# blackjax-devs/blackjax

Measured on AMD Instinct MI355X. Metric: chain-leapfrog-steps/sec (whole node), 65 536 chains x 1 024-dim diag-mass HMC, higher is better.
Workload: dtype f32

## Files before the change

blackjax_amd/_lib.py:

```python
from __future__ import annotations

import ctypes
import os
from ctypes import POINTER, c_char_p, c_float, c_int, c_int64, c_uint32, c_void_p

_HERE = os.path.dirname(os.path.abspath(__file__))
LIB_PATH = os.path.join(_HERE, "libbjxhip.so")

_f32p = c_void_p
_u8p = c_void_p

SIGNATURES = {
    "bjx_abi_version": [],
    "bjx_keys_split": [c_uint32, c_uint32, c_int64, c_int64, POINTER(c_uint32)],
    "bjx_rng_normal": [c_void_p, c_uint32, c_uint32, c_int64, c_int64, c_int64, _f32p],
    "bjx_rng_uniform": [c_void_p, c_uint32, c_uint32, c_int64, c_int64, _f32p],
    "bjx_rng_key_probe": [c_void_p, c_uint32, c_uint32, c_int64, _f32p, _f32p, c_int64, c_void_p],
    "bjx_log1p_device_check": [c_void_p, c_uint32, c_void_p],
    "bjx_hmc_momentum_diag": [c_void_p, c_uint32, c_uint32, c_int64, c_int64, c_int64, c_int64, _f32p,
                              c_int64, _f32p, _f32p],
    "bjx_hmc_momentum_kick_diag": [c_void_p, c_uint32, c_uint32, c_int64, c_int64, c_int64, c_int64, _f32p,
                                   c_int64, c_float, _f32p, _f32p, _f32p, _f32p, _f32p, _f32p, _f32p],
    "bjx_leapfrog_diag": [c_void_p, c_int64, c_int64, c_int, c_float, _f32p, _f32p, c_int64,
                          _f32p, _f32p, _f32p, _f32p, _f32p],
# ... 62 lines not shown
                                 _f32p, _f32p, _f32p, _f32p, _f32p, _u8p, _u8p, _f32p, _f32p, _f32p, _f32p,
                                 _f32p, c_void_p],
    "bjx_pc_matvec_t": [c_void_p, c_int64, c_int64, _f32p, c_int64, _f32p, _f32p],
    "bjx_hmc_momentum_dense_pc": [c_void_p, c_uint32, c_uint32, c_int64, c_int64, c_int64, c_int64,
                                  _f32p, _f32p, c_int64, _f32p, _f32p, _f32p, _f32p],
    "bjx_leapfrog_dense_pc": [c_void_p, c_int64, c_int64, c_int, c_float, _f32p, _f32p, c_int64, _f32p,
                              _f32p, _f32p, _f32p, _f32p],
    "bjx_hmc_finish_dense_pc": [c_void_p, c_uint32, c_uint32, c_int64, c_int64, c_int64, c_int64,
                                c_float, _f32p, _f32p, c_int64, c_float,
                                _f32p, _f32p, _f32p, _f32p, _f32p, _f32p, _f32p, _f32p,
                                _f32p, _f32p, _f32p, _f32p, _f32p, _f32p, _f32p, _u8p, _u8p, _f32p],
    "bjx_welford_update_dense": [c_void_p, c_int64, c_int64, c_int64, _f32p, _f32p, _f32p, _f32p,
                                 _f32p],
    "bjx_welford_final_dense": [c_void_p, c_int64, c_int64, c_int64, c_float, _f32p, _f32p, c_int,
                                _f32p],
    "bjx_da_init": [c_void_p, c_int64, c_int, _f32p, _f32p, _f32p, _f32p, _f32p, _f32p],
    "bjx_da_update": [c_void_p, c_int64, c_int64, c_float, c_float, c_float, c_float, _f32p, _f32p,
                      _f32p, _f32p, _f32p, _f32p, _f32p, _f32p, _f32p],
    "bjx_exp": [c_void_p, c_int64, _f32p, _f32p],
    "bjx_welford_update_diag": [c_void_p, c_int64, c_int64, c_int64, _f32p, _f32p, _f32p, _f32p, _f32p],
    "bjx_welford_final_diag": [c_void_p, c_int64, c_int64, c_int64, c_float, _f32p, _f32p, c_int64,
                               _f32p],
    "bjx_target_diag_gaussian": [c_void_p, c_int64, c_int64, _f32p, _f32p, _f32p, _f32p],
    "bjx_target_neal_funnel": [c_void_p, c_int64, c_int64, _f32p, _f32p, _f32p],
    "bjx_target_ar1_gaussian": [c_void_p, c_int64, c_int64, c_float, c_float, c_float, _f32p,
                                _f32p, _f32p],
}



class NutsDesc(ctypes.Structure):

    _fields_ = [
        ("N", c_int64), ("D", c_int64), ("max_depth", ctypes.c_int32), ("reserved", ctypes.c_int32),
        ("imm", c_void_p), ("imm_stride", c_int64), ("eps_per_chain", c_void_p),
        ("eps", c_float), ("divergence_threshold", c_float),
        ("key0", c_uint32), ("key1", c_uint32), ("chain_offset", c_int64), ("step_fold", c_int64),
        ("q0", c_void_p), ("g0", c_void_p), ("p0", c_void_p),
        ("Lq", c_void_p), ("Lp", c_void_p), ("Lg", c_void_p),
        ("Rq", c_void_p), ("Rp", c_void_p), ("Rg", c_void_p),
        ("msum", c_void_p), ("Smsum", c_void_p),
        ("Pq", c_void_p), ("Pg", c_void_p), ("Sq", c_void_p), ("Sg", c_void_p),
        ("ckpt_r", c_void_p), ("ckpt_rs", c_void_p),
        ("fs", c_void_p), ("is_", c_void_p),
        ("Mdense", c_void_p), ("Mdense_stride", c_int64), ("v0", c_void_p),
        ("Lv", c_void_p), ("Rv", c_void_p), ("ckpt_v", c_void_p),
# ... 235 lines not shown
```

blackjax_amd/_util.py:

```python
from __future__ import annotations

import threading
import weakref
from typing import Callable

import torch

_VG_CACHE: "weakref.WeakKeyDictionary" = weakref.WeakKeyDictionary()
_CAPTURE_LOCK = threading.RLock()
_CAPTURE_TLS = threading.local()
_GRAVEYARD: list = []


class LockedGraph(torch.cuda.CUDAGraph):

    def __del__(self):
        try:
            if getattr(_CAPTURE_TLS, "depth", 0) > 0:
                _GRAVEYARD.append(self)
                return
            with _CAPTURE_LOCK:
                self.reset()
        except Exception:
            pass
# ... 94 lines not shown
                    return lp_a, g_a
            return tgt(q)
        lp, g = first if first is not None else _autograd(q)
        ew[key] = _try_elementwise(logdensity_fn, q, lp, g)
        return lp, g

    def vg(q):
        if mode["kind"] == "autograd":
            return _autograd_or_elementwise(q)
        if mode["kind"] == "pair":
            return logdensity_fn(q)
        qg = q.detach().requires_grad_(True)
        with torch.enable_grad():
            out = logdensity_fn(qg)
            if isinstance(out, (tuple, list)) and len(out) == 2:
                mode["kind"] = "pair"
                lp, g = out[0].detach(), out[1].detach()
                del out
                return lp, g
            mode["kind"] = "autograd"
            g = _grad(out, qg)
        return _autograd_or_elementwise(q, first=(out.detach(), g))

    vg._bjx_elementwise = ew
    vg._bjx_value_and_grad = True
    try:
        _VG_CACHE[logdensity_fn] = vg
    except TypeError:
        pass
    return vg


_WARNED_AUTOGRAD: set = set()
_RECHECK_AT = (16, 256)
_RECHECK_EVERY = 4096


def _close(a, b) -> bool:
    a, b = a.float(), b.float()
    fin = torch.isfinite(b)
    scale = float(b[fin].abs().max()) if bool(fin.any()) else 1.0
    same_nonfinite = bool(((a == b) | (torch.isnan(a) & torch.isnan(b)))[~fin].all())
    return same_nonfinite and bool(((a - b)[fin].abs() <= 1e-4 * max(scale, 1e-30)).all())


def no_trace(logdensity_fn: Callable) -> Callable:
# ... 114 lines not shown
        raise RuntimeError(
            f"{name} lives on {x.device}: blackjax_amd runs on ROCm device tensors only "
            "(there is no CPU fallback)"
        )
    if x.dtype != torch.float32:
        raise TypeError(f"{name} must be float32, got {x.dtype}")
    return x.contiguous()


def eval_logdensity(vg: Callable, q: torch.Tensor):
    logp, g = vg(q)
    if logp.dtype != torch.float32:
        logp = logp.float()
    if g.dtype != torch.float32:
        g = g.float()
    if g.shape != q.shape or logp.shape != q.shape[:1]:
        raise ValueError(
            f"logdensity_fn must return logp of shape {tuple(q.shape[:1])} and grad of shape "
            f"{tuple(q.shape)}; got {tuple(logp.shape)} and {tuple(g.shape)}"
        )
    return logp.contiguous(), g.contiguous()


def step_size_args(step_size, n_chains: int, device):
    if isinstance(step_size, torch.Tensor):
        if step_size.ndim == 0 and not step_size.is_cuda:
            return float(step_size), None
        t = step_size.to(device=device, dtype=torch.float32)
        if t.ndim == 0:
            t = t.expand(n_chains)
        if t.shape != (n_chains,):
            raise ValueError(f"per-chain step_size must have shape ({n_chains},), got {tuple(t.shape)}")
        return 0.0, t.contiguous()
    return float(step_size), None
```

blackjax_amd/csrc/bjx_targets.hip:

```cpp
#include "../../include/bjx_hip.h"
#include "bjx_device.h"
#include "bjx_host.h"
#include "bjx_targets_dev.h"

using namespace bjx;

namespace {

constexpr int kBlock = 256;
constexpr int kWavesPerBlock = kBlock / BJX_WAVE;

__device__ __forceinline__ int64_t wave_row0() {
  return (int64_t)blockIdx.x * kWavesPerBlock + (threadIdx.x >> 6);
}
__device__ __forceinline__ int64_t wave_row_stride() { return (int64_t)gridDim.x * kWavesPerBlock; }

template <int VEC, bool NT = false>
__global__ void __launch_bounds__(kBlock)
k_diag_gaussian(int64_t N, int64_t D, const float* __restrict__ iv, const float* __restrict__ q,
                float* __restrict__ logp, float* __restrict__ g) {
  const int lane = threadIdx.x & 63;
  for (int64_t r = wave_row0(); r < N; r += wave_row_stride()) {
    const int64_t base = r * D;
    double acc = 0.0;
// ... 15 lines not shown
          if (j < D) {
            F4 gg{-(qq[u].x * vv[u].x), -(qq[u].y * vv[u].y), -(qq[u].z * vv[u].z), -(qq[u].w * vv[u].w)};
            acc += (double)qq[u].x * (double)gg.x;
            acc += (double)qq[u].y * (double)gg.y;
            acc += (double)qq[u].z * (double)gg.z;
            acc += (double)qq[u].w * (double)gg.w;
            st4_t<NT>(g + base + j, gg);
          }
        }
      }
    } else {
      for (int64_t j = lane; j < D; j += 64) {
        const float qq = q[base + j];
        const float gg = -(qq * iv[j]);
        acc += (double)qq * (double)gg;
        g[base + j] = gg;
      }
    }
    acc = wave_sum(acc);
    if (lane == 0) logp[r] = (float)(0.5 * acc);
  }
}

template <int G>
__global__ void __launch_bounds__(kBlock)
k_diag_gaussian_short(int64_t N, int64_t D, const float* __restrict__ iv, const float* __restrict__ q,
                      float* __restrict__ logp, float* __restrict__ g) {
  constexpr int R = BJX_WAVE / G;
  const int lane = threadIdx.x & 63;
  const int sub = lane / G, gl = lane % G;
  for (int64_t r0 = wave_row0() * R; r0 < N; r0 += wave_row_stride() * R) {
    const int64_t r = r0 + sub;
    const bool valid = r < N;
    double acc = 0.0;
    if (valid) {
      const int64_t base = r * D;
      for (int64_t j = (int64_t)gl * 4; j < D; j += G * 4) {
        const F4 qq = ld4(q + base + j), vv = ld4(iv + j);
        const F4 gg{-(qq.x * vv.x), -(qq.y * vv.y), -(qq.z * vv.z), -(qq.w * vv.w)};
        acc += (double)qq.x * (double)gg.x;
        acc += (double)qq.y * (double)gg.y;
        acc += (double)qq.z * (double)gg.z;
        acc += (double)qq.w * (double)gg.w;
        st4(g + base + j, gg);
      }
    }
// ... 87 lines not shown
    hipLaunchKernelGGL(k_diag_gaussian_short<8>, dim3(bjx_row_grid((N + 7) / 8, kWavesPerBlock)), block, 0,
                       (hipStream_t)stream, N, D, inv_var, q, logp_out, g_out);
  else if (bjx_vec4_ok(D, inv_var, q, g_out) && D <= 64)
    hipLaunchKernelGGL(k_diag_gaussian_short<16>, dim3(bjx_row_grid((N + 3) / 4, kWavesPerBlock)), block, 0,
                       (hipStream_t)stream, N, D, inv_var, q, logp_out, g_out);
  else if (bjx_vec4_ok(D, inv_var, q, g_out) && D <= 128)
    hipLaunchKernelGGL(k_diag_gaussian_short<32>, dim3(bjx_row_grid((N + 1) / 2, kWavesPerBlock)), block, 0,
                       (hipStream_t)stream, N, D, inv_var, q, logp_out, g_out);
  else if (bjx_vec4_ok(D, inv_var, q, g_out)) {
    static const int nt_mode = [] { const char* e = getenv("BJX_LF_NT"); return e ? atoi(e) : -1; }();
    const bool nt = nt_mode < 0 ? N * D * 8 > ((int64_t)256 << 20) : nt_mode != 0;
    if (nt)
      hipLaunchKernelGGL((k_diag_gaussian<4, true>), grid, block, 0, (hipStream_t)stream, N, D, inv_var, q,
                         logp_out, g_out);
    else
      hipLaunchKernelGGL((k_diag_gaussian<4, false>), grid, block, 0, (hipStream_t)stream, N, D, inv_var, q,
                         logp_out, g_out);
  } else
    hipLaunchKernelGGL(k_diag_gaussian<1>, grid, block, 0, (hipStream_t)stream, N, D, inv_var, q,
                       logp_out, g_out);
  return bjx_check_launch("bjx_target_diag_gaussian");
}

int bjx_target_neal_funnel(void* stream, int64_t N, int64_t D, const float* q, float* logp_out,
                           float* g_out) {
  BJX_CHECK_ARG(N >= 0 && D >= 2, "bjx_target_neal_funnel: bad arguments");
  if (N == 0) return 0;
  BJX_CHECK_ARG(q && logp_out && g_out, "bjx_target_neal_funnel: bad arguments");
  const dim3 grid(bjx_row_grid(N, kWavesPerBlock));
  hipStream_t st = (hipStream_t)stream;
  if (bjx_vec4_ok(D, q, g_out) && D <= 1024) {
    const dim3 wgrid((unsigned)(N < ((int64_t)1 << 20) ? N : ((int64_t)1 << 20)));
    if (D <= 256) hipLaunchKernelGGL(k_neal_funnel_v4<1>, wgrid, dim3(64), 0, st, N, D, q, logp_out, g_out);
    else if (D <= 512) hipLaunchKernelGGL(k_neal_funnel_v4<2>, wgrid, dim3(64), 0, st, N, D, q, logp_out, g_out);
    else hipLaunchKernelGGL(k_neal_funnel_v4<4>, wgrid, dim3(64), 0, st, N, D, q, logp_out, g_out);
  } else {
    hipLaunchKernelGGL(k_neal_funnel, grid, dim3(kBlock), 0, st, N, D, q, logp_out, g_out);
  }
  return bjx_check_launch("bjx_target_neal_funnel");
}

int bjx_target_ar1_gaussian(void* stream, int64_t N, int64_t D, float diag_edge, float diag_mid,
                            float off, const float* q, float* logp_out, float* g_out) {
  BJX_CHECK_ARG(N >= 0 && D >= 2, "bjx_target_ar1_gaussian: bad arguments");
  if (N == 0) return 0;
  BJX_CHECK_ARG(q && logp_out && g_out, "bjx_target_ar1_gaussian: bad arguments");
// ... 7 lines not shown
```

blackjax_amd/csrc/bjx_traj_dev.h:

```cpp
#pragma once

#include "bjx_device.h"
#include "bjx_targets_dev.h"

namespace bjx {

struct TrajArgs {
  Key key;
  int64_t off, fold, N, D, L;
  float eps_s;
  const float* eps_pc;
  const float* imm;
  int64_t imm_stride;
  float thr;
  const float* params;
  const float *q0, *logp0, *g0;
  float *p0_out, *q1_out, *p_end_out, *logp1_out, *g1_out;
  float *q_out, *logp_out, *g_out, *acc_rate_out, *energy_out;
  uint8_t *is_acc_out, *is_div_out;
};

static_assert(sizeof(TrajArgs) == 216, "blackjax_amd/rtc.py mirrors this struct field for field (TrajArgs)");

struct FunnelTarget {
// ... 151 lines not shown
  }
}

template <int NI, class Target>
__device__ __forceinline__ void target_rows(int64_t N, int64_t D, const float* params, const float* q,
                                            float* logp, float* grad) {
  const int lane = threadIdx.x & 63;
  const int waves = blockDim.x >> 6;
  for (int64_t r = (int64_t)blockIdx.x * waves + (threadIdx.x >> 6); r < N; r += (int64_t)gridDim.x * waves) {
    typename Target::template Ctx<NI> ctx;
    Target::template init<NI>(ctx, D, params);
    F4 x[NI], g[NI];
    float lp = 0.0f;
#pragma unroll
    for (int k = 0; k < NI; ++k) {
      const int64_t j = ((int64_t)lane + 64 * k) * 4;
      if (j < D) x[k] = ld4(q + r * D + j);
    }
    Target::template eval<NI>(ctx, D, params, x, true, g, lp);
    target_store<NI>(D, g, lp, logp + r, grad + r * D);
  }
}

}
```

blackjax_amd/elementwise.py:

```python
from __future__ import annotations

import math
import operator
from typing import Callable

import torch

__all__ = ["from_elementwise", "ElementwiseSource"]


class _E:

    __slots__ = ("v", "d")

    def __init__(self, v: str, d):
        self.v, self.d = v, d


class _R:

    __slots__ = ("coef", "const")

    def __init__(self, coef: dict, const: float = 0.0):
        self.coef, self.const = coef, float(const)
# ... 358 lines not shown
          const float xs[4] = {{xq[u].x, xq[u].y, xq[u].z, xq[u].w}}; {p_unpack_u}
          float gs[4];
#pragma unroll
          for (int e = 0; e < 4; ++e) {{
            const float x = xs[e]; {p_decl}
            {body}
            gs[e] = {g_expr};
            {acc_add_rows}
          }}
          st4(gr + j, F4{{gs[0], gs[1], gs[2], gs[3]}});
        }});
    }} else {{
      for (int64_t j = lane; j < D; j += 64) {{
        const float x = qr[j]; {p_scalar}
        {body}
        gr[j] = {g_expr};
        {acc_add_rows}
      }}
    }}
    const float lp = (float)({lp_expr});
    if (lane == 0) logp[r] = lp;
  }}
}}
"""
    params = torch.stack(gen.params).contiguous() if gen.params else None
    src = ElementwiseSource(source, params, len(used),
                            f"{len(gen.lines)} fp32 ops per element, {n_p} parameter vector(s), {len(used)} row sum(s)")
    src.rows_source = rows_source
    return src


class _Wrap(torch.nn.Module):

    def __init__(self, fn):
        super().__init__()
        self._fn = fn

    def forward(self, q):
        return self._fn(q)


ROWS_TU = """#include "bjx_traj_dev.h"
using namespace bjx;
%(source)s
"""

# ... 14 lines not shown
```

blackjax_amd/hmc.py:

```python
from __future__ import annotations

from typing import Callable, NamedTuple

import torch

from . import _lib, integrators, metrics
from ._util import (new_graph, record_graph, check_batch, eval_logdensity, is_capturable, step_size_args, value_and_grad,
                    warn_eager_driver)
from .base import SamplingAlgorithm
from .random import key_spec

__all__ = ["HMCState", "HMCInfo", "IntegratorState", "init", "flip_momentum", "build_kernel", "as_top_level_api"]


class HMCState(NamedTuple):

    position: torch.Tensor
    logdensity: torch.Tensor
    logdensity_grad: torch.Tensor


class IntegratorState(NamedTuple):

    position: torch.Tensor
    momentum: torch.Tensor
    logdensity: torch.Tensor
    logdensity_grad: torch.Tensor


class HMCInfo(NamedTuple):

# ... 161 lines not shown
    return int(v)


_IC_WORKING_SET_BYTES = 192 << 20


def auto_chain_block(n_chains: int, dim: int, arrays: int = 3) -> int:
    blk = (_IC_WORKING_SET_BYTES // (4 * int(arrays) * max(int(dim), 1))) // 1024 * 1024
    if blk < 1024 or blk >= n_chains:
        return int(n_chains)
    return int(blk)


class _GraphedTrajectory:

    def __init__(self, n, D, L, vg, imm_per_chain, device, owner=None):
        self.n, self.D, self.L = n, D, L
        self.owner = owner
        self.Wq = torch.empty((n, D), dtype=torch.float32, device=device)
        self.Wp = torch.empty((n, D), dtype=torch.float32, device=device)
        self.eps = torch.ones(n, dtype=torch.float32, device=device)
        self.imm = torch.ones((n, D) if imm_per_chain else (D,), dtype=torch.float32, device=device)
        self.imm_stride = D if imm_per_chain else 0
        self.Wq.zero_()
        self.Wp.zero_()
        self._vg = vg
        side = torch.cuda.Stream(device=device)
        side.wait_stream(torch.cuda.current_stream(device))
        with torch.cuda.stream(side):
            self._body()
        torch.cuda.current_stream(device).wait_stream(side)
        torch.cuda.synchronize(device)
        self.graph = new_graph()
        with record_graph(self.graph):
            self.logp, self.g = self._body()

    def _body(self):
        stream = _lib.current_stream()
        logp, g = eval_logdensity(self._vg, self.Wq)
        for _ in range(self.L - 1):
            _lib.call("bjx_leapfrog_diag", stream, self.n, self.D, 2, 0.0, self.eps.data_ptr(),
                      self.imm.data_ptr(), self.imm_stride, self.Wq.data_ptr(), self.Wp.data_ptr(),
                      g.data_ptr(), self.Wq.data_ptr(), self.Wp.data_ptr())
            del logp, g
            logp, g = eval_logdensity(self._vg, self.Wq)
        return logp, g


_SIDE_STREAMS: dict = {}


def _side_streams(dev, n):
    pool = _SIDE_STREAMS.setdefault(dev.index, [])
    while len(pool) < n:
        pool.append(torch.cuda.Stream(device=dev))
    return pool[:n]


def build_kernel(integrator=integrators.velocity_verlet, divergence_threshold: float = 1000,
                 build_proposal=None, *, chain_block=None, use_graph="auto", streams="auto"):
    if use_graph not in (True, False, "auto"):
        raise ValueError("use_graph must be True, False or 'auto'")
    thr = float(divergence_threshold)
    if build_proposal is multinomial_hmc_proposal:
        integrators.check_supported(integrator, allow_general=True)
        return _build_mhmc_kernel(thr, integrator.coefficients[0::2], integrator.coefficients[1::2])
    if build_proposal not in (None, hmc_proposal):
        raise NotImplementedError(
# ... 50 lines not shown
                cb = N
        blk = N if not cb or cb >= N else int(cb)
        n_blocks = (N + blk - 1) // blk if N else 0
        fn_id = id(logdensity_fn)
        if (use_graph == "auto" and L >= 2 and N > 0 and metric.kind == "diag" and not general
                and blk * D <= (1 << 21) and is_capturable(logdensity_fn)
                and fn_id not in not_capturable):
            gkey = (min(blk, N), D, L, fn_id, metric.imm_stride != 0, dev.index)
            seen[gkey] = seen.get(gkey, 0) + 1
            try:
                if gkey not in graphs and seen[gkey] >= 2 and len(graphs) < 8:
                    graphs[gkey] = _GraphedTrajectory(min(blk, N), D, L, vg, metric.imm_stride != 0, dev,
                                                      owner=logdensity_fn)
                graphed = gkey in graphs
            except RuntimeError:
                not_capturable[fn_id] = logdensity_fn
                torch.cuda.synchronize(dev)
        if (use_graph == "auto" and L >= 2 and N > 0 and metric.kind == "diag" and not general
                and blk * D <= (1 << 21) and not is_capturable(logdensity_fn)):
            warn_eager_driver(logdensity_fn, "hmc")
        single = n_blocks <= 1 and not graphed
        q_end = torch.empty_like(q0) if L > 0 else q0
        p_work = torch.empty_like(q0) if (L > 0 and not graphed) else None
        g_end = torch.empty_like(q0) if (L > 0 and not single) else None
        logp_end = torch.empty_like(logp0) if (L > 0 and not single) else None
        if L == 0:
            g_end, logp_end = g0, logp0

        def block_args(b):
            s, e = b * blk, min(N, (b + 1) * blk)
            sl = slice(s, e)
            if metric.kind == "dense_pc":
                m = metric._replace(imm=metric.imm[sl], mass_sqrt_t=metric.mass_sqrt_t[sl])
            else:
                m = metric if metric.imm_stride == 0 else metric._replace(imm=metric.imm[sl])
            return e - s, sl, m, (None if eps_pc is None else eps_pc[sl]), off + s

        fused_first = (metric.kind == "diag" and L > 0 and not graphed and not general and D > 128 and _FUSE_FIRST)

        def launch_first(b, stream_):
            n, sl, m, eb, boff = block_args(b)
            _lib.call("bjx_hmc_momentum_kick_diag", stream_, k0, k1, boff, fold, n, D, m.imm.data_ptr(),
                      m.imm_stride, eps, _lib.ptr(eb), q0[sl].data_ptr(), g0[sl].data_ptr(),
                      p0[sl].data_ptr(), ke0[sl].data_ptr(), q_end[sl].data_ptr(), p_work[sl].data_ptr())

        def run_block(b):
            nonlocal g_end, logp_end
            stream = _lib.current_stream()
            n, sl, m, eb, boff = block_args(b)
            if fused_first:
                q, p = q_end[sl], p_work[sl]
                launch_first(b, stream)
            elif m.kind == "diag":
                _lib.call("bjx_hmc_momentum_diag", stream, k0, k1, boff, fold, n, D, m.imm.data_ptr(),
                          m.imm_stride, p0[sl].data_ptr(), ke0[sl].data_ptr())
            else:
                from . import dense

                dense.momentum(stream, m, k0, k1, boff, fold, n, D, p0[sl], ke0[sl])

            if L == 0:
                q, p, logp, g = q0[sl], p0[sl], logp0[sl], g0[sl]
                eps_fin, eps_pc_fin = 0.0, None
            elif graphed:
                gkey = (n, D, L, fn_id, m.imm_stride != 0, dev.index)
                ctx = graphs.get(gkey)
                if ctx is None:
                    ctx = graphs[gkey] = _GraphedTrajectory(n, D, L, vg, m.imm_stride != 0, dev,
                                                            owner=logdensity_fn)
                if eb is None:
                    ctx.eps.fill_(eps)
                else:
                    ctx.eps.copy_(eb)
                ctx.imm.copy_(m.imm)
                _launch_leapfrog(stream, m, n, D, 1, eps, eb, q0[sl], p0[sl], g0[sl], ctx.Wq, ctx.Wp)
                ctx.graph.replay()
                q, p, logp, g = ctx.Wq, ctx.Wp, ctx.logp, ctx.g
                eps_fin, eps_pc_fin = eps, eb
            elif general:
                q, p = q_end[sl], p_work[sl]

                def stage(n_k, ka, kb, a_c, q_in, p_in, g_in, p_out):
                    if m.kind == "diag":
                        _lib.call("bjx_leapfrog_diag_coef", stream, n, D, n_k, ka, kb, a_c, eps, _lib.ptr(eb),
                                  m.imm.data_ptr(), m.imm_stride, q_in.data_ptr(), p_in.data_ptr(),
                                  g_in.data_ptr(), q.data_ptr(), p_out.data_ptr(), None, 0)
                        return p_out
                    from . import dense

                    return dense.leapfrog_coef(stream, m, n, D, n_k, ka, kb, a_c, eps, eb, q_in, p_in,
                                               g_in, q, p_out)

                first = True
                for _ in range(L):
                    for si, a_c in enumerate(drift_c):
                        if first:
                            p = stage(1, kick_c[0], 0.0, a_c, q0[sl], p0[sl], g0[sl], p)
                            first = False
                        elif si == 0:
                            p = stage(2, kick_c[-1], kick_c[0], a_c, q, p, g, p)
                        else:
                            p = stage(1, kick_c[si], 0.0, a_c, q, p, g, p)
                        logp, g = eval_logdensity(vg, q)
                        yield
                        stream = _lib.current_stream()
                eps_fin, eps_pc_fin = eps, eb
            else:
                if not fused_first:
                    q, p = q_end[sl], p_work[sl]
                    p = _launch_leapfrog(stream, m, n, D, 1, eps, eb, q0[sl], p0[sl], g0[sl], q, p)
                logp, g = eval_logdensity(vg, q)
                for _ in range(L - 1):
                    yield
                    stream = _lib.current_stream()
                    p = _launch_leapfrog(stream, m, n, D, 2, eps, eb, q, p, g, q, p)
                    logp, g = eval_logdensity(vg, q)
                yield
                stream = _lib.current_stream()
                eps_fin, eps_pc_fin = eps, eb

            if m.kind == "diag" and general:
                _lib.call("bjx_hmc_finish_diag_coef", stream, k0, k1, boff, fold, n, D, kick_c[-1],
                          eps_fin, _lib.ptr(eps_pc_fin), m.imm.data_ptr(), m.imm_stride, thr,
                          q0[sl].data_ptr(), logp0[sl].data_ptr(), g0[sl].data_ptr(),
                          ke0[sl].data_ptr(), q.data_ptr(), logp.data_ptr(), g.data_ptr(),
                          p.data_ptr(), p_end[sl].data_ptr(), q_new[sl].data_ptr(),
                          logp_new[sl].data_ptr(), g_new[sl].data_ptr(), acc_rate[sl].data_ptr(),
                          is_acc[sl].data_ptr(), is_div[sl].data_ptr(), energy[sl].data_ptr())
            elif m.kind == "diag":
                _lib.call("bjx_hmc_finish_diag", stream, k0, k1, boff, fold, n, D, eps_fin,
                          _lib.ptr(eps_pc_fin), m.imm.data_ptr(), m.imm_stride, thr,
                          q0[sl].data_ptr(), logp0[sl].data_ptr(), g0[sl].data_ptr(),
                          ke0[sl].data_ptr(), q.data_ptr(), logp.data_ptr(), g.data_ptr(),
                          p.data_ptr(), p_end[sl].data_ptr(), q_new[sl].data_ptr(),
                          logp_new[sl].data_ptr(), g_new[sl].data_ptr(), acc_rate[sl].data_ptr(),
                          is_acc[sl].data_ptr(), is_div[sl].data_ptr(), energy[sl].data_ptr())
            elif general:
                from . import dense

                dense.finish_coef(stream, m, k0, k1, boff, fold, n, D, kick_c[-1], eps_fin, eps_pc_fin, thr,
                                  q0[sl], logp0[sl], g0[sl], ke0[sl], q, logp, g, p, p_end[sl], q_new[sl],
                                  logp_new[sl], g_new[sl], acc_rate[sl], is_acc[sl], is_div[sl], energy[sl])
            else:
                from . import dense

                dense.finish(stream, m, k0, k1, boff, fold, n, D, eps_fin, eps_pc_fin, thr, q0[sl],
                             logp0[sl], g0[sl], ke0[sl], q, logp, g, p, p_end[sl], q_new[sl],
                             logp_new[sl], g_new[sl], acc_rate[sl], is_acc[sl], is_div[sl],
                             energy[sl])
            if L > 0:
                if single:
                    g_end, logp_end = g, logp
                else:
                    g_end[sl].copy_(g)
                    logp_end[sl].copy_(logp)
                    if graphed:
                        q_end[sl].copy_(q)


        ns = 1 if (graphed or n_blocks <= 1) else min(int(n_streams), n_blocks)
        if ns <= 1:
            for b in range(n_blocks):
                for _ in run_block(b):
                    pass
        else:
            main = torch.cuda.current_stream(dev)
            pool = _side_streams(dev, ns)
            for st_ in pool:
                st_.wait_stream(main)
            for w0 in range(0, n_blocks, ns):
                active = [(run_block(b), pool[b - w0]) for b in range(w0, min(w0 + ns, n_blocks))]
                while active:
                    for item in list(active):
                        with torch.cuda.stream(item[1]):
                            try:
                                next(item[0])
                            except StopIteration:
                                active.remove(item)
            for st_ in pool:
                main.wait_stream(st_)
# ... 87 lines not shown
```

blackjax_amd/rtc.py:

```python
from __future__ import annotations

import ctypes
import os

_HERE = os.path.dirname(os.path.abspath(__file__))
CSRC = os.path.join(_HERE, "csrc")
ARCH = "gfx950"

_rtc = None
_hip = None


def _librtc():
    global _rtc
    if _rtc is None:
        _rtc = ctypes.CDLL("libhiprtc.so")
        _rtc.hiprtcGetErrorString.restype = ctypes.c_char_p
    return _rtc


def _libhip():
    global _hip
    if _hip is None:
        _hip = ctypes.CDLL("libamdhip64.so")
# ... 79 lines not shown
                ("L", ctypes.c_int64), ("eps_s", ctypes.c_float), ("eps_pc", ctypes.c_void_p),
                ("imm", ctypes.c_void_p), ("imm_stride", ctypes.c_int64), ("thr", ctypes.c_float),
                ("params", ctypes.c_void_p), ("q0", ctypes.c_void_p), ("logp0", ctypes.c_void_p),
                ("g0", ctypes.c_void_p), ("p0_out", ctypes.c_void_p), ("q1_out", ctypes.c_void_p),
                ("p_end_out", ctypes.c_void_p), ("logp1_out", ctypes.c_void_p), ("g1_out", ctypes.c_void_p),
                ("q_out", ctypes.c_void_p), ("logp_out", ctypes.c_void_p), ("g_out", ctypes.c_void_p),
                ("acc_rate_out", ctypes.c_void_p), ("energy_out", ctypes.c_void_p),
                ("is_acc_out", ctypes.c_void_p), ("is_div_out", ctypes.c_void_p)]


TARGET_TU = """#include "bjx_traj_dev.h"
using namespace bjx;
// ---- user source
%(source)s
// ---- kernels around it
#define BJX_RTC_KERNELS(NI_)                                                                              \\
  extern "C" __global__ void __launch_bounds__(256) bjx_rtc_traj_##NI_(TrajArgs a) {                      \\
    hmc_trajectory_rows<NI_, %(struct)s>(a);                                                              \\
  }                                                                                                       \\
  extern "C" __global__ void __launch_bounds__(256) bjx_rtc_eval_##NI_(long long N, long long D,          \\
                                                                       const float* params, const float* q, \\
                                                                       float* logp, float* grad) {        \\
    target_rows<NI_, %(struct)s>(N, D, params, q, logp, grad);                                            \\
  }
BJX_RTC_KERNELS(1)
BJX_RTC_KERNELS(2)
BJX_RTC_KERNELS(4)
"""


def ni_for(dim: int) -> int:
    return 1 if dim <= 256 else (2 if dim <= 512 else 4)


NUTS_TU = """#include "bjx_traj_dev.h"
using namespace bjx;
// ---- user source
%(source)s
// ---- the engine's NUTS device code around it
#define BJX_RTC_USER_TARGET %(struct)s
#include "bjx_nuts_tick_dev.h"
#define BJX_RTC_NUTS(NI_, FULL_, NAME_)                                                                      \\
  extern "C" __global__ void __launch_bounds__(64) __attribute__((amdgpu_waves_per_eu(2)))                   \\
  NAME_(bjx_nuts_t nt, bjx_nuts_async_t ax, float* qf, float* logp_f, float* gf) {                           \\
    const int64_t n_rows = async_n_rows(ax);                                                                 \\
    for (int64_t b = blockIdx.x; b < n_rows; b += gridDim.x)                                                 \\
# ... 13 lines not shown
```

blackjax_amd/targets.py:

```python
from __future__ import annotations

import numpy as np
import torch

from . import _lib
from ._util import check_batch


class _Target:
    _bjx_value_and_grad = True
    _bjx_returns_pair = True
    _bjx_capturable = True

    def _alloc(self, q):
        q = check_batch(q, "q")
        return q, torch.empty(q.shape[0], dtype=torch.float32, device=q.device), torch.empty_like(q)


class DiagGaussian(_Target):
    def __init__(self, inv_var: torch.Tensor):
        self.inv_var = check_batch(inv_var, "inv_var")

    def _bjx_fused_target(self, dim: int):
        if dim > 128 and tuple(self.inv_var.shape) == (dim,):
            return 2, self.inv_var
        return None

    def __call__(self, q):
        q, logp, g = self._alloc(q)
        N, D = q.shape
        if self.inv_var.shape != (D,):
            raise ValueError(f"inv_var has shape {tuple(self.inv_var.shape)}, expected ({D},)")
        _lib.call("bjx_target_diag_gaussian", _lib.current_stream(), N, D, self.inv_var.data_ptr(),
                  q.data_ptr(), logp.data_ptr(), g.data_ptr())
        return logp, g


class NealFunnel(_Target):
    def _bjx_fused_target(self, dim: int):
        return 1, None

    def __call__(self, q):
        q, logp, g = self._alloc(q)
        N, D = q.shape
        _lib.call("bjx_target_neal_funnel", _lib.current_stream(), N, D, q.data_ptr(),
                  logp.data_ptr(), g.data_ptr())
        return logp, g


class AR1Gaussian(_Target):
    def __init__(self, rho: float, dim: int):
        self.rho, self.dim = float(rho), int(dim)
        c = np.float32(1.0 / (1.0 - self.rho * self.rho))
        self.d_edge = float(np.float32(1.0) * c)
        self.d_mid = float(np.float32(1.0 + self.rho * self.rho) * c)
        self.off = float(np.float32(-self.rho) * c)

    def covariance(self, device) -> torch.Tensor:
        i = torch.arange(self.dim, device=device)
        return (self.rho ** (i[:, None] - i[None, :]).abs().double()).float()

    def __call__(self, q):
        q, logp, g = self._alloc(q)
        N, D = q.shape
        if D != self.dim:
            raise ValueError(f"expected dim {self.dim}, got {D}")
        _lib.call("bjx_target_ar1_gaussian", _lib.current_stream(), N, D, self.d_edge, self.d_mid,
                  self.off, q.data_ptr(), logp.data_ptr(), g.data_ptr())
        return logp, g


class DeviceTarget(_Target):

    def __init__(self, source: str, params: torch.Tensor | None = None, struct: str = "Target"):
        self.source, self.struct = str(source), str(struct)
        if params is not None:
            if not (isinstance(params, torch.Tensor) and params.dtype == torch.float32 and params.is_contiguous()):
                raise ValueError("params must be a contiguous float32 tensor")
        self.params = params
        self._code = None
        self._module = None

    def code_object(self) -> bytes:
        if self._code is None:
            from . import rtc

            self._code = rtc.compile(rtc.TARGET_TU % {"source": self.source, "struct": self.struct},
                                     f"bjx_device_target_{self.struct}.hip")
        return self._code

    def module(self):
        if self._module is None:
            from . import rtc

            self._module = rtc.Module(self.code_object())
        return self._module

    def nuts_module(self):
        if getattr(self, "_nuts_module", None) is None:
            from . import rtc

            self._nuts_module = rtc.Module(rtc.compile(rtc.NUTS_TU % {"source": self.source, "struct": self.struct},
                                                       f"bjx_device_target_nuts_{self.struct}.hip"))
        return self._nuts_module

    def _params_ptr(self, device):
        if self.params is None:
            return 0
        if self.params.device != device:
            raise ValueError(f"params live on {self.params.device}, the chains on {device}")
        return self.params.data_ptr()

    def _bjx_fused_target(self, dim: int):
        return ("rtc", self) if dim % 4 == 0 and dim <= 1024 else None

    def __call__(self, q):
        import ctypes

        from . import rtc

        q, logp, g = self._alloc(q)
        N, D = q.shape
        if D % 4 != 0 or D > 1024:
            raise ValueError("DeviceTarget: rows of at most 1 024 floats, a multiple of 4")
        if N == 0:
            return logp, g
        grid = min((N + 3) // 4, 1 << 20)
        self.module().launch(f"bjx_rtc_eval_{rtc.ni_for(D)}", grid, 256, _lib.current_stream(),
                             ctypes.c_longlong(N), ctypes.c_longlong(D), ctypes.c_void_p(self._params_ptr(q.device)),
                             ctypes.c_void_p(q.data_ptr()), ctypes.c_void_p(logp.data_ptr()),
                             ctypes.c_void_p(g.data_ptr()))
        return logp, g


class ElementwiseRowsTarget(_Target):

    def __init__(self, src, dim: int):
        self.elementwise, self.dim = src, int(dim)
        self.params = src.params
        self._module = None

    def code_object(self) -> bytes:
        from . import elementwise, rtc

        return rtc.compile(elementwise.ROWS_TU % {"source": self.elementwise.rows_source}, "bjx_elementwise_rows.hip")

    def module(self):
        if self._module is None:
            from . import rtc

            self._module = rtc.Module(self.code_object())
        return self._module

    def _bjx_fused_target(self, dim: int):
        return None

    def __call__(self, q):
        import ctypes

        q, logp, g = self._alloc(q)
        N, D = q.shape
        if D != self.dim:
            raise ValueError(f"this target was generated for D = {self.dim}, got {D}")
        if N == 0:
            return logp, g
        if self.params is not None and self.params.device != q.device:
            raise ValueError(f"params live on {self.params.device}, the chains on {q.device}")
        grid = min((N + 3) // 4, 1 << 20)
        self.module().launch("bjx_rtc_ew_rows", grid, 256, _lib.current_stream(), ctypes.c_longlong(N),
                             ctypes.c_longlong(D), ctypes.c_void_p(0 if self.params is None else self.params.data_ptr()),
                             ctypes.c_void_p(q.data_ptr()), ctypes.c_void_p(logp.data_ptr()), ctypes.c_void_p(g.data_ptr()))
        return logp, g


def from_elementwise(fn, dim: int, device="cuda"):
    from .elementwise import from_elementwise as _f

    return _f(fn, dim, device)
```

include/bjx_hip.h:

```cpp
#ifndef BJX_HIP_H
#define BJX_HIP_H

#include <stdint.h>

#ifdef __cplusplus
extern "C" {
#endif

#define BJX_ABI_VERSION 7

const char* bjx_last_error(void);
int bjx_abi_version(void);

int bjx_keys_split(uint32_t key0, uint32_t key1, int64_t n, int64_t offset, uint32_t* out);

int bjx_rng_normal(void* stream, uint32_t key0, uint32_t key1, int64_t chain_offset,
                   int64_t N, int64_t D, float* z_out);
int bjx_rng_uniform(void* stream, uint32_t key0, uint32_t key1, int64_t chain_offset,
                    int64_t N, float* u_out);
int bjx_rng_key_probe(void* stream, uint32_t key0, uint32_t key1, int64_t D, float* z_out, float* u_out,
                      int64_t n_children, uint32_t* children_out);

int bjx_log1p_device_check(void* stream, uint32_t stride, unsigned long long* counts_out);

// ... 189 lines not shown
                            int imm_prev_per_chain, float* imm_out);

int bjx_da_init(void* stream, int64_t N, int from_log_avg, const float* x_in, float* log_x_out,
                float* log_x_avg_out, float* avg_error_out, float* mu_out, float* step_size_out);

int bjx_da_update(void* stream, int64_t N, int64_t step, float target, float t0, float gamma,
                  float kappa, const float* acceptance_rate, const float* log_x_in,
                  const float* log_x_avg_in, const float* avg_error_in, const float* mu,
                  float* log_x_out, float* log_x_avg_out, float* avg_error_out,
                  float* step_size_out);

int bjx_exp(void* stream, int64_t N, const float* x, float* y);

int bjx_welford_update_diag(void* stream, int64_t N, int64_t D, int64_t sample_size_new,
                            const float* value, const float* mean_in, const float* m2_in,
                            float* mean_out, float* m2_out);

int bjx_welford_final_diag(void* stream, int64_t N, int64_t D, int64_t sample_size,
                           float imm_shrinkage_to_previous, const float* m2, const float* imm_prev,
                           int64_t imm_prev_stride, float* imm_out);

int bjx_target_diag_gaussian(void* stream, int64_t N, int64_t D, const float* inv_var,
                             const float* q, float* logp_out, float* g_out);
int bjx_target_neal_funnel(void* stream, int64_t N, int64_t D, const float* q,
                           float* logp_out, float* g_out);
int bjx_target_ar1_gaussian(void* stream, int64_t N, int64_t D, float diag_edge,
                            float diag_mid, float off, const float* q, float* logp_out,
                            float* g_out);

#ifdef __cplusplus
}
#endif

#include "bjx_nuts.h"

#endif
```

Before: 233.2 million.

## Evaluate gradient-only targets into preallocated buffers during leapfrog trajectories

Adds gradient-only target kernels (diag Gaussian, RTC device targets, elementwise targets) and an eval_into path that writes logp/grad into preallocated buffers. Intermediate leapfrog steps skip the logp row reduction and per-call tensor allocation, and the final copy into g_end is avoided. The diag Gaussian grad kernel uses flat vec4 launches with optional nontemporal loads/stores and a reversed workgroup ordering within groups of 8. The change adds more code paths and extra gating checks per call.

```diff
diff --git a/blackjax_amd/_lib.py b/blackjax_amd/_lib.py
--- a/blackjax_amd/_lib.py
+++ b/blackjax_amd/_lib.py
@@ -108,6 +108,7 @@
     "bjx_welford_final_diag": [c_void_p, c_int64, c_int64, c_int64, c_float, _f32p, _f32p, c_int64,
                                _f32p],
     "bjx_target_diag_gaussian": [c_void_p, c_int64, c_int64, _f32p, _f32p, _f32p, _f32p],
+    "bjx_target_diag_gaussian_grad": [c_void_p, c_int64, c_int64, _f32p, _f32p, _f32p],
     "bjx_target_neal_funnel": [c_void_p, c_int64, c_int64, _f32p, _f32p, _f32p],
     "bjx_target_ar1_gaussian": [c_void_p, c_int64, c_int64, c_float, c_float, c_float, _f32p,
                                 _f32p, _f32p],
diff --git a/blackjax_amd/_util.py b/blackjax_amd/_util.py
--- a/blackjax_amd/_util.py
+++ b/blackjax_amd/_util.py
@@ -140,6 +140,30 @@
             g = _grad(out, qg)
         return _autograd_or_elementwise(q, first=(out.detach(), g))
 
+    def _generated(q):
+        if mode["kind"] != "autograd":
+            return None
+        key = (int(q.shape[-1]), q.device)
+        tgt = ew.get(key)
+        if tgt is None:
+            return None
+        n = calls.get(key, 0) + 1
+        if (n in _RECHECK_AT or n % _RECHECK_EVERY == 0) and not (q.is_cuda and torch.cuda.is_current_stream_capturing()):
+            return None
+        calls[key] = n
+        return tgt
+
+    def eval_into_(q, logp_out, g_out):
+        tgt = _generated(q)
+        return False if tgt is None else tgt._bjx_eval_into(q, logp_out, g_out)
+
+    def grad_into_(q, g_out):
+        tgt = _generated(q)
+        return False if tgt is None else tgt._bjx_grad_into(q, g_out)
+
+    if mode["kind"] != "pair":
+        vg._bjx_eval_into = eval_into_
+        vg._bjx_grad_into = grad_into_
     vg._bjx_elementwise = ew
     vg._bjx_value_and_grad = True
     try:
@@ -300,6 +324,17 @@
     return logp.contiguous(), g.contiguous()
 
 
+def eval_into(vg: Callable, q: torch.Tensor, logp_out: torch.Tensor, g_out: torch.Tensor, need_logp: bool = True):
+    if not need_logp:
+        f = getattr(vg, "_bjx_grad_into", None)
+        if f is not None and f(q, g_out) is not False:
+            return None, g_out
+    f = getattr(vg, "_bjx_eval_into", None)
+    if f is not None and f(q, logp_out, g_out) is not False:
+        return logp_out, g_out
+    return eval_logdensity(vg, q)
+
+
 def step_size_args(step_size, n_chains: int, device):
     if isinstance(step_size, torch.Tensor):
         if step_size.ndim == 0 and not step_size.is_cuda:
diff --git a/blackjax_amd/csrc/bjx_targets.hip b/blackjax_amd/csrc/bjx_targets.hip
--- a/blackjax_amd/csrc/bjx_targets.hip
+++ b/blackjax_amd/csrc/bjx_targets.hip
@@ -61,6 +61,50 @@
   }
 }
 
+#ifndef BJX_REVERSE_ROWS
+#define BJX_REVERSE_ROWS 1
+#endif
+
+__device__ __forceinline__ unsigned grad_span_of_workgroup() {
+  const unsigned b = blockIdx.x, G = gridDim.x;
+  if (!BJX_REVERSE_ROWS || (b | 7u) >= G) return b;
+  return (b & ~7u) + ((G - 1u - b) & 7u);
+}
+
+template <bool NT = false>
+__global__ void __launch_bounds__(kBlock)
+k_diag_gaussian_grad_flat(int64_t D, int bpr, const float* __restrict__ iv, const float* __restrict__ q,
+                          float* __restrict__ g) {
+  const unsigned b = grad_span_of_workgroup();
+  const int64_t r = b / (unsigned)bpr;
+  const int64_t j = (int64_t)(b - (unsigned)r * (unsigned)bpr) * 1024 + threadIdx.x * 4;
+  const int64_t at = r * D + j;
+  const F4 qq = ld4_t<NT>(q + at), vv = ld4(iv + j);
+  st4_t<NT>(g + at, F4{-(qq.x * vv.x), -(qq.y * vv.y), -(qq.z * vv.z), -(qq.w * vv.w)});
+}
+
+template <bool NT = false>
+__global__ void __launch_bounds__(kBlock)
+k_diag_gaussian_grad_flat_any(uint32_t total4, uint32_t D4, const float* __restrict__ iv,
+                              const float* __restrict__ q, float* __restrict__ g) {
+  const uint32_t i = grad_span_of_workgroup() * kBlock + threadIdx.x;
+  if (i >= total4) return;
+  const uint32_t j4 = i % D4;
+  const int64_t at = (int64_t)i * 4;
+  const F4 qq = ld4_t<NT>(q + at), vv = ld4(iv + (int64_t)j4 * 4);
+  st4_t<NT>(g + at, F4{-(qq.x * vv.x), -(qq.y * vv.y), -(qq.z * vv.z), -(qq.w * vv.w)});
+}
+
+__global__ void __launch_bounds__(kBlock)
+k_diag_gaussian_grad_rows(int64_t N, int64_t D, const float* __restrict__ iv, const float* __restrict__ q,
+                          float* __restrict__ g) {
+  const int lane = threadIdx.x & 63;
+  for (int64_t r = wave_row0(); r < N; r += wave_row_stride()) {
+    const int64_t base = r * D;
+    for (int64_t j = lane; j < D; j += 64) g[base + j] = -(q[base + j] * iv[j]);
+  }
+}
+
 template <int G>
 __global__ void __launch_bounds__(kBlock)
 k_diag_gaussian_short(int64_t N, int64_t D, const float* __restrict__ iv, const float* __restrict__ q,
@@ -194,6 +238,33 @@
   return bjx_check_launch("bjx_target_diag_gaussian");
 }
 
+int bjx_target_diag_gaussian_grad(void* stream, int64_t N, int64_t D, const float* inv_var, const float* q,
+                                  float* g_out) {
+  BJX_CHECK_ARG(N >= 0 && D > 0, "bjx_target_diag_gaussian_grad: bad arguments");
+  if (N == 0) return 0;
+  BJX_CHECK_ARG(inv_var && q && g_out, "bjx_target_diag_gaussian_grad: bad arguments");
+  const dim3 block(kBlock);
+  hipStream_t s = (hipStream_t)stream;
+  static const int nt_mode = [] { const char* e = getenv("BJX_LF_NT"); return e ? atoi(e) : -1; }();
+  const bool nt = nt_mode < 0 ? N * D * 8 > ((int64_t)256 << 20) : nt_mode != 0;
+  const bool v4 = bjx_vec4_ok(D, inv_var, q, g_out);
+  if (v4 && D % 1024 == 0 && N * (D / 1024) < ((int64_t)1 << 31)) {
+    const int bpr = (int)(D / 1024);
+    const dim3 grid((unsigned)(N * bpr));
+    if (nt) hipLaunchKernelGGL(k_diag_gaussian_grad_flat<true>, grid, block, 0, s, D, bpr, inv_var, q, g_out);
+    else hipLaunchKernelGGL(k_diag_gaussian_grad_flat<false>, grid, block, 0, s, D, bpr, inv_var, q, g_out);
+  } else if (v4 && N * (D / 4) < ((int64_t)1 << 31)) {
+    const uint32_t D4 = (uint32_t)(D / 4), total4 = (uint32_t)(N * (D / 4));
+    const dim3 grid((total4 + kBlock - 1) / kBlock);
+    if (nt) hipLaunchKernelGGL(k_diag_gaussian_grad_flat_any<true>, grid, block, 0, s, total4, D4, inv_var, q, g_out);
+    else hipLaunchKernelGGL(k_diag_gaussian_grad_flat_any<false>, grid, block, 0, s, total4, D4, inv_var, q, g_out);
+  } else {
+    hipLaunchKernelGGL(k_diag_gaussian_grad_rows, dim3(bjx_row_grid(N, kWavesPerBlock)), block, 0, s, N, D,
+                       inv_var, q, g_out);
+  }
+  return bjx_check_launch("bjx_target_diag_gaussian_grad");
+}
+
 int bjx_target_neal_funnel(void* stream, int64_t N, int64_t D, const float* q, float* logp_out,
                            float* g_out) {
   BJX_CHECK_ARG(N >= 0 && D >= 2, "bjx_target_neal_funnel: bad arguments");
diff --git a/blackjax_amd/csrc/bjx_traj_dev.h b/blackjax_amd/csrc/bjx_traj_dev.h
--- a/blackjax_amd/csrc/bjx_traj_dev.h
+++ b/blackjax_amd/csrc/bjx_traj_dev.h
@@ -197,4 +197,28 @@
   }
 }
 
-}
+template <int NI, class Target>
+__device__ __forceinline__ void target_grad_rows(int64_t N, int64_t D, const float* params, const float* q,
+                                                 float* grad) {
+  const int lane = threadIdx.x & 63;
+  const int waves = blockDim.x >> 6;
+  for (int64_t r = (int64_t)blockIdx.x * waves + (threadIdx.x >> 6); r < N; r += (int64_t)gridDim.x * waves) {
+    typename Target::template Ctx<NI> ctx;
+    Target::template init<NI>(ctx, D, params);
+    F4 x[NI], g[NI];
+    float lp = 0.0f;
+#pragma unroll
+    for (int k = 0; k < NI; ++k) {
+      const int64_t j = ((int64_t)lane + 64 * k) * 4;
+      if (j < D) x[k] = ld4(q + r * D + j);
+    }
+    Target::template eval<NI>(ctx, D, params, x, false, g, lp);
+#pragma unroll
+    for (int k = 0; k < NI; ++k) {
+      const int64_t j = ((int64_t)lane + 64 * k) * 4;
+      if (j < D) st4(grad + r * D + j, g[k]);
+    }
+  }
+}
+
+}
diff --git a/blackjax_amd/elementwise.py b/blackjax_amd/elementwise.py
--- a/blackjax_amd/elementwise.py
+++ b/blackjax_amd/elementwise.py
@@ -404,6 +404,39 @@
     if (lane == 0) logp[r] = lp;
   }}
 }}
+
+// the gradient alone: the same element-wise body without the row sums (a trajectory's intermediate evaluations)
+extern "C" __global__ void __launch_bounds__(256) bjx_rtc_ew_grad_rows(long long N, long long D, const float* __restrict__ params,
+                                                                        const float* __restrict__ q, float* __restrict__ grad) {{
+  const int lane = threadIdx.x & 63;
+  const int waves = blockDim.x >> 6;
+  for (int64_t r = (int64_t)blockIdx.x * waves + (threadIdx.x >> 6); r < N; r += (int64_t)gridDim.x * waves) {{
+    const float* qr = q + r * D;
+    float* gr = grad + r * D;
+    if (D % 4 == 0) {{
+      F4 xq[4]; {p_decl_arr}
+      row_sweep4<4>(lane, D,
+        [&](int u, int64_t j) {{ xq[u] = ld4(qr + j); {p_load_u}}},
+        [&](int u, int64_t j) {{
+          const float xs[4] = {{xq[u].x, xq[u].y, xq[u].z, xq[u].w}}; {p_unpack_u}
+          float gs[4];
+#pragma unroll
+          for (int e = 0; e < 4; ++e) {{
+            const float x = xs[e]; {p_decl}
+            {body}
+            gs[e] = {g_expr};
+          }}
+          st4(gr + j, F4{{gs[0], gs[1], gs[2], gs[3]}});
+        }});
+    }} else {{
+      for (int64_t j = lane; j < D; j += 64) {{
+        const float x = qr[j]; {p_scalar}
+        {body}
+        gr[j] = {g_expr};
+      }}
+    }}
+  }}
+}}
 """
     params = torch.stack(gen.params).contiguous() if gen.params else None
     src = ElementwiseSource(source, params, len(used),
diff --git a/blackjax_amd/hmc.py b/blackjax_amd/hmc.py
--- a/blackjax_amd/hmc.py
+++ b/blackjax_amd/hmc.py
@@ -5,8 +5,8 @@
 import torch
 
 from . import _lib, integrators, metrics
-from ._util import (new_graph, record_graph, check_batch, eval_logdensity, is_capturable, step_size_args, value_and_grad,
-                    warn_eager_driver)
+from ._util import (new_graph, record_graph, check_batch, eval_into, eval_logdensity, is_capturable, step_size_args,
+                    value_and_grad, warn_eager_driver)
 from .base import SamplingAlgorithm
 from .random import key_spec
 
@@ -214,6 +214,8 @@
         self.eps = torch.ones(n, dtype=torch.float32, device=device)
         self.imm = torch.ones((n, D) if imm_per_chain else (D,), dtype=torch.float32, device=device)
         self.imm_stride = D if imm_per_chain else 0
+        self._g = torch.empty((n, D), dtype=torch.float32, device=device)
+        self._logp = torch.empty(n, dtype=torch.float32, device=device)
         self.Wq.zero_()
         self.Wp.zero_()
         self._vg = vg
@@ -229,13 +231,13 @@
 
     def _body(self):
         stream = _lib.current_stream()
-        logp, g = eval_logdensity(self._vg, self.Wq)
-        for _ in range(self.L - 1):
+        logp, g = eval_into(self._vg, self.Wq, self._logp, self._g, need_logp=self.L == 1)
+        for i in range(self.L - 1):
             _lib.call("bjx_leapfrog_diag", stream, self.n, self.D, 2, 0.0, self.eps.data_ptr(),
                       self.imm.data_ptr(), self.imm_stride, self.Wq.data_ptr(), self.Wp.data_ptr(),
                       g.data_ptr(), self.Wq.data_ptr(), self.Wp.data_ptr())
             del logp, g
-            logp, g = eval_logdensity(self._vg, self.Wq)
+            logp, g = eval_into(self._vg, self.Wq, self._logp, self._g, need_logp=i == self.L - 2)
         return logp, g
 
 
@@ -332,8 +334,9 @@
         single = n_blocks <= 1 and not graphed
         q_end = torch.empty_like(q0) if L > 0 else q0
         p_work = torch.empty_like(q0) if (L > 0 and not graphed) else None
-        g_end = torch.empty_like(q0) if (L > 0 and not single) else None
-        logp_end = torch.empty_like(logp0) if (L > 0 and not single) else None
+        writes_into = getattr(vg, "_bjx_eval_into", None) is not None
+        g_end = torch.empty_like(q0) if (L > 0 and (not single or writes_into)) else None
+        logp_end = torch.empty_like(logp0) if (L > 0 and (not single or writes_into)) else None
         if L == 0:
             g_end, logp_end = g0, logp0
 
@@ -358,6 +361,16 @@
             nonlocal g_end, logp_end
             stream = _lib.current_stream()
             n, sl, m, eb, boff = block_args(b)
+            if L > 0 and g_end is not None:
+                g_buf, logp_buf = (g_end, logp_end) if single else (g_end[sl], logp_end[sl])
+            else:
+                g_buf = logp_buf = None
+
+            def evaluate(q_, need_logp):
+                if g_buf is None:
+                    return eval_logdensity(vg, q_)
+                return eval_into(vg, q_, logp_buf, g_buf, need_logp)
+
             if fused_first:
                 q, p = q_end[sl], p_work[sl]
                 launch_first(b, stream)
@@ -402,7 +415,8 @@
                                                g_in, q, p_out)
 
                 first = True
-                for _ in range(L):
+                logp = g = None
+                for i in range(L):
                     for si, a_c in enumerate(drift_c):
                         if first:
                             p = stage(1, kick_c[0], 0.0, a_c, q0[sl], p0[sl], g0[sl], p)
@@ -411,7 +425,8 @@
                             p = stage(2, kick_c[-1], kick_c[0], a_c, q, p, g, p)
                         else:
                             p = stage(1, kick_c[si], 0.0, a_c, q, p, g, p)
-                        logp, g = eval_logdensity(vg, q)
+                        del logp, g
+                        logp, g = evaluate(q, i == L - 1 and si == len(drift_c) - 1)
                         yield
                         stream = _lib.current_stream()
                 eps_fin, eps_pc_fin = eps, eb
@@ -419,12 +434,13 @@
                 if not fused_first:
                     q, p = q_end[sl], p_work[sl]
                     p = _launch_leapfrog(stream, m, n, D, 1, eps, eb, q0[sl], p0[sl], g0[sl], q, p)
-                logp, g = eval_logdensity(vg, q)
-                for _ in range(L - 1):
+                logp, g = evaluate(q, L == 1)
+                for i in range(L - 1):
                     yield
                     stream = _lib.current_stream()
                     p = _launch_leapfrog(stream, m, n, D, 2, eps, eb, q, p, g, q, p)
-                    logp, g = eval_logdensity(vg, q)
+                    del logp, g
+                    logp, g = evaluate(q, i == L - 2)
                 yield
                 stream = _lib.current_stream()
                 eps_fin, eps_pc_fin = eps, eb
@@ -459,13 +475,15 @@
                              logp_new[sl], g_new[sl], acc_rate[sl], is_acc[sl], is_div[sl],
                              energy[sl])
             if L > 0:
-                if single:
+                if g is g_buf:
+                    pass
+                elif single:
                     g_end, logp_end = g, logp
                 else:
                     g_end[sl].copy_(g)
                     logp_end[sl].copy_(logp)
-                    if graphed:
-                        q_end[sl].copy_(q)
+                if graphed:
+                    q_end[sl].copy_(q)
 
 
         ns = 1 if (graphed or n_blocks <= 1) else min(int(n_streams), n_blocks)
diff --git a/blackjax_amd/rtc.py b/blackjax_amd/rtc.py
--- a/blackjax_amd/rtc.py
+++ b/blackjax_amd/rtc.py
@@ -125,6 +125,11 @@
                                                                        const float* params, const float* q, \\
                                                                        float* logp, float* grad) {        \\
     target_rows<NI_, %(struct)s>(N, D, params, q, logp, grad);                                            \\
+  }                                                                                                       \\
+  extern "C" __global__ void __launch_bounds__(256) bjx_rtc_grad_##NI_(long long N, long long D,          \\
+                                                                       const float* params, const float* q, \\
+                                                                       float* grad) {                     \\
+    target_grad_rows<NI_, %(struct)s>(N, D, params, q, grad);                                             \\
   }
 BJX_RTC_KERNELS(1)
 BJX_RTC_KERNELS(2)
diff --git a/blackjax_amd/targets.py b/blackjax_amd/targets.py
--- a/blackjax_amd/targets.py
+++ b/blackjax_amd/targets.py
@@ -16,6 +16,11 @@
         q = check_batch(q, "q")
         return q, torch.empty(q.shape[0], dtype=torch.float32, device=q.device), torch.empty_like(q)
 
+    def __call__(self, q):
+        q, logp, g = self._alloc(q)
+        self._bjx_eval_into(q, logp, g)
+        return logp, g
+
 
 class DiagGaussian(_Target):
     def __init__(self, inv_var: torch.Tensor):
@@ -26,26 +31,29 @@
             return 2, self.inv_var
         return None
 
-    def __call__(self, q):
-        q, logp, g = self._alloc(q)
+    def _bjx_eval_into(self, q, logp, g):
         N, D = q.shape
         if self.inv_var.shape != (D,):
             raise ValueError(f"inv_var has shape {tuple(self.inv_var.shape)}, expected ({D},)")
         _lib.call("bjx_target_diag_gaussian", _lib.current_stream(), N, D, self.inv_var.data_ptr(),
                   q.data_ptr(), logp.data_ptr(), g.data_ptr())
-        return logp, g
+
+    def _bjx_grad_into(self, q, g):
+        N, D = q.shape
+        if self.inv_var.shape != (D,):
+            raise ValueError(f"inv_var has shape {tuple(self.inv_var.shape)}, expected ({D},)")
+        _lib.call("bjx_target_diag_gaussian_grad", _lib.current_stream(), N, D, self.inv_var.data_ptr(),
+                  q.data_ptr(), g.data_ptr())
 
 
 class NealFunnel(_Target):
     def _bjx_fused_target(self, dim: int):
         return 1, None
 
-    def __call__(self, q):
-        q, logp, g = self._alloc(q)
+    def _bjx_eval_into(self, q, logp, g):
         N, D = q.shape
         _lib.call("bjx_target_neal_funnel", _lib.current_stream(), N, D, q.data_ptr(),
                   logp.data_ptr(), g.data_ptr())
-        return logp, g
 
 
 class AR1Gaussian(_Target):
@@ -60,14 +68,12 @@
         i = torch.arange(self.dim, device=device)
         return (self.rho ** (i[:, None] - i[None, :]).abs().double()).float()
 
-    def __call__(self, q):
-        q, logp, g = self._alloc(q)
+    def _bjx_eval_into(self, q, logp, g):
         N, D = q.shape
         if D != self.dim:
             raise ValueError(f"expected dim {self.dim}, got {D}")
         _lib.call("bjx_target_ar1_gaussian", _lib.current_stream(), N, D, self.d_edge, self.d_mid,
                   self.off, q.data_ptr(), logp.data_ptr(), g.data_ptr())
-        return logp, g
 
 
 class DeviceTarget(_Target):
@@ -114,23 +120,26 @@
     def _bjx_fused_target(self, dim: int):
         return ("rtc", self) if dim % 4 == 0 and dim <= 1024 else None
 
-    def __call__(self, q):
+    def _launch_rows(self, kernel, q, *outs):
         import ctypes
 
         from . import rtc
 
-        q, logp, g = self._alloc(q)
         N, D = q.shape
         if D % 4 != 0 or D > 1024:
             raise ValueError("DeviceTarget: rows of at most 1 024 floats, a multiple of 4")
         if N == 0:
-            return logp, g
+            return
         grid = min((N + 3) // 4, 1 << 20)
-        self.module().launch(f"bjx_rtc_eval_{rtc.ni_for(D)}", grid, 256, _lib.current_stream(),
+        self.module().launch(f"{kernel}_{rtc.ni_for(D)}", grid, 256, _lib.current_stream(),
                              ctypes.c_longlong(N), ctypes.c_longlong(D), ctypes.c_void_p(self._params_ptr(q.device)),
-                             ctypes.c_void_p(q.data_ptr()), ctypes.c_void_p(logp.data_ptr()),
-                             ctypes.c_void_p(g.data_ptr()))
-        return logp, g
+                             ctypes.c_void_p(q.data_ptr()), *[ctypes.c_void_p(t.data_ptr()) for t in outs])
+
+    def _bjx_eval_into(self, q, logp, g):
+        self._launch_rows("bjx_rtc_eval", q, logp, g)
+
+    def _bjx_grad_into(self, q, g):
+        self._launch_rows("bjx_rtc_grad", q, g)
 
 
 class ElementwiseRowsTarget(_Target):
@@ -155,22 +164,26 @@
     def _bjx_fused_target(self, dim: int):
         return None
 
-    def __call__(self, q):
+    def _launch_rows(self, kernel, q, *outs):
         import ctypes
 
-        q, logp, g = self._alloc(q)
         N, D = q.shape
         if D != self.dim:
             raise ValueError(f"this target was generated for D = {self.dim}, got {D}")
         if N == 0:
-            return logp, g
+            return
         if self.params is not None and self.params.device != q.device:
             raise ValueError(f"params live on {self.params.device}, the chains on {q.device}")
         grid = min((N + 3) // 4, 1 << 20)
-        self.module().launch("bjx_rtc_ew_rows", grid, 256, _lib.current_stream(), ctypes.c_longlong(N),
+        self.module().launch(kernel, grid, 256, _lib.current_stream(), ctypes.c_longlong(N),
                              ctypes.c_longlong(D), ctypes.c_void_p(0 if self.params is None else self.params.data_ptr()),
-                             ctypes.c_void_p(q.data_ptr()), ctypes.c_void_p(logp.data_ptr()), ctypes.c_void_p(g.data_ptr()))
-        return logp, g
+                             ctypes.c_void_p(q.data_ptr()), *[ctypes.c_void_p(t.data_ptr()) for t in outs])
+
+    def _bjx_eval_into(self, q, logp, g):
+        self._launch_rows("bjx_rtc_ew_rows", q, logp, g)
+
+    def _bjx_grad_into(self, q, g):
+        self._launch_rows("bjx_rtc_ew_grad_rows", q, g)
 
 
 def from_elementwise(fn, dim: int, device="cuda"):
diff --git a/include/bjx_hip.h b/include/bjx_hip.h
--- a/include/bjx_hip.h
+++ b/include/bjx_hip.h
@@ -235,6 +235,8 @@
 
 int bjx_target_diag_gaussian(void* stream, int64_t N, int64_t D, const float* inv_var,
                              const float* q, float* logp_out, float* g_out);
+int bjx_target_diag_gaussian_grad(void* stream, int64_t N, int64_t D, const float* inv_var,
+                                  const float* q, float* g_out);
 int bjx_target_neal_funnel(void* stream, int64_t N, int64_t D, const float* q,
                            float* logp_out, float* g_out);
 int bjx_target_ar1_gaussian(void* stream, int64_t N, int64_t D, float diag_edge,
```

Measured after the change: 243.5 million, median of 6. 4.4% higher.
